# linuxstb/dabtools

Hardware: AMD Instinct MI355X
Metric: ETI frames/s (24 ms each), Mode-I batch, synthetic IQ resident in HBM (higher is better)
Workload: dtype f64 sync / f32 OFDM / u16 ACS / u8 ETI

## Files before the change

### dabtools_amd/csrc/fft64.hpp

```cpp
#pragma once

#include <hip/hip_runtime.h>

namespace dabhip {
namespace {

constexpr int kFft64Threads = 512;

__device__ __forceinline__ unsigned brev(unsigned x, int bits) { return __brev(x) >> (32 - bits); }

__device__ __forceinline__ int lds_at(int i) { return i ^ ((i >> 3) & 7) ^ ((i >> 6) & 7); }

template <class V>
struct ScalarOf;
template <>
struct ScalarOf<double2> { using type = double; };
template <>
struct ScalarOf<float2> { using type = float; };

template <int LOGN, int L, class V>
__device__ __forceinline__ void dif_levels(V* buf, int nbatch, int s, typename ScalarOf<V>::type sign, const V* tw2048)
{
  using R = typename ScalarOf<V>::type;
  constexpr int N = 1 << LOGN, RADIX = 1 << L;
  const int ms = N >> s;
  const int q = ms >> L;
  constexpr int per_batch = N >> L;
  for (int idx = threadIdx.x; idx < nbatch * per_batch; idx += kFft64Threads) {
    const int batch = idx / per_batch, w = idx % per_batch;
    const int blk = w / q, k = w % q;
    const int e0 = batch * N + blk * ms + k;
    V r[RADIX];
#pragma unroll
    for (int j = 0; j < RADIX; ++j) r[j] = buf[lds_at(e0 + j * q)];
#pragma unroll
    for (int l = 0; l < L; ++l) {
      const int span = RADIX >> (l + 1);
      const int half = ms >> (l + 1);
      const int twstep = 1024 / half;
#pragma unroll
      for (int j = 0; j < RADIX; ++j) {
        if (j & span) continue;
        const int pos = k + (j & (span - 1)) * q;
        const V A = r[j], B = r[j + span];
        V tw = tw2048[lds_at(pos * twstep)];
        tw.y *= sign;
        const R dr = A.x - B.x, di = A.y - B.y;
        r[j].x = A.x + B.x;
        r[j].y = A.y + B.y;
        r[j + span].x = dr * tw.x - di * tw.y;
        r[j + span].y = dr * tw.y + di * tw.x;
      }
    }
#pragma unroll
    for (int j = 0; j < RADIX; ++j) buf[lds_at(e0 + j * q)] = r[j];
  }
  __syncthreads();
}

template <int LOGN, int... Ls, class V>
__device__ __forceinline__ void dft_dif(V* buf, int nbatch, typename ScalarOf<V>::type sign, const V* tw2048)
{
  int s = 0;
  ((dif_levels<LOGN, Ls>(buf, nbatch, s, sign, tw2048), s += Ls), ...);
}

}
}
```

### dabtools_amd/csrc/k_sync.hip

```cpp
#include <hip/hip_runtime.h>

#include <algorithm>
#include <cstdlib>
#include <type_traits>

#include "dab_tables.hpp"
#include "device_types.hpp"
#include "fft64.hpp"
#include "fifo_view.hpp"
#include "kernels.hpp"

namespace dabhip {
namespace {

constexpr int kThreads = kFft64Threads;

#ifndef DABHIP_SYNC_TIMES
#define DABHIP_SYNC_TIMES 0
#endif
#ifndef DABHIP_K1_TAIL
#define DABHIP_K1_TAIL 1
#endif
#if DABHIP_SYNC_TIMES
__device__ unsigned long long g_sync_times[96 * 16];
__device__ volatile int g_sync_call;
#define SYNC_STAMP(i) do { if (blockIdx.x == 0 && threadIdx.x == 0 && g_sync_call < 96) g_sync_times[g_sync_call * 16 + (i)] = wall_clock64(); } while (0)
#else
#define SYNC_STAMP(i) do {} while (0)
#endif

__device__ __forceinline__ int view_byte(const uint8_t* stream, const FrameView& v, int p) { return frame_byte(stream, v, p); }
__device__ __forceinline__ double2 view_sample(const uint8_t* stream, const FrameView& v, int p, int nco_hz)
{
  const unsigned w = frame_u16(stream, v, p);
  const double2 x = make_double2(static_cast<int8_t>(static_cast<uint8_t>((w & 0xff) - 127)), static_cast<int8_t>(static_cast<uint8_t>((w >> 8) - 127)));
  if (nco_hz == 0) return x;
  double sn, cs;
  sincospi(-2.0 * nco_hz * (p >> 1) / 2048000.0, &sn, &cs);
  return make_double2(x.x * cs - x.y * sn, x.x * sn + x.y * cs);
}
__device__ __forceinline__ int rail(int byte) { return static_cast<int>(static_cast<int8_t>(static_cast<uint8_t>(byte - 127))); }

__device__ __forceinline__ const uint8_t* contiguous_window(const uint8_t* stream, const FrameView& v, int p0, int p1)
{
  return (v.seg_src[0] >= 0 && p1 <= v.seg_end[0]) ? stream + v.seg_src[0] + p0 : nullptr;
}
__device__ __forceinline__ double2 sample_of(unsigned w)
{
  return make_double2(static_cast<int8_t>(static_cast<uint8_t>((w & 0xff) - 127)), static_cast<int8_t>(static_cast<uint8_t>((w >> 8) - 127)));
}
template <int kCount>
struct Prefetched {
  bool ok;
  unsigned w[kCount / kThreads];
};
template <int kCount>
__device__ __forceinline__ Prefetched<kCount> prefetch_samples(const uint8_t* stream, const FrameView& view, int p0, int nco)
{
  Prefetched<kCount> pf;
  const uint8_t* win = nco == 0 ? contiguous_window(stream, view, p0, p0 + 2 * kCount) : nullptr;
  pf.ok = win != nullptr;
  if (pf.ok) {
    const uint16_t* src = reinterpret_cast<const uint16_t*>(win);
#pragma unroll
    for (int i = 0; i < kCount / kThreads; ++i) pf.w[i] = src[threadIdx.x + i * kThreads];
  }
  return pf;
}
template <int kCount>
__device__ __forceinline__ void load_samples(const uint8_t* stream, const FrameView& view, int p0, int nco, double2* dst)
{
  const int tid = threadIdx.x;
  const uint8_t* win = nco == 0 ? contiguous_window(stream, view, p0, p0 + 2 * kCount) : nullptr;
  if (win) {
    const uint16_t* src = reinterpret_cast<const uint16_t*>(win);
    unsigned w[kCount / kThreads];
#pragma unroll
    for (int i = 0; i < kCount / kThreads; ++i) w[i] = src[tid + i * kThreads];
#pragma unroll
    for (int i = 0; i < kCount / kThreads; ++i) dst[lds_at(tid + i * kThreads)] = sample_of(w[i]);
  } else {
    for (int n = tid; n < kCount; n += kThreads) dst[lds_at(n)] = view_sample(stream, view, p0 + 2 * n, nco);
  }
}

constexpr int kWaves = kThreads / 64;
struct Red {
  float fv[kWaves];
  int iv[kWaves];
  double dv[kWaves];
};

template <int kCtrl, int kRowMask>
__device__ __forceinline__ int dpp_from(int own)
{
  return __builtin_amdgcn_update_dpp(own, own, kCtrl, kRowMask, 0xf, false);
}
template <typename F>
__device__ __forceinline__ void wave_reduce_steps(F&& step)
{
  step(std::integral_constant<int, 0xB1>{}, std::integral_constant<int, 0xf>{});
  step(std::integral_constant<int, 0x4E>{}, std::integral_constant<int, 0xf>{});
  step(std::integral_constant<int, 0x141>{}, std::integral_constant<int, 0xf>{});
  step(std::integral_constant<int, 0x140>{}, std::integral_constant<int, 0xf>{});
  step(std::integral_constant<int, 0x142>{}, std::integral_constant<int, 0xa>{});
  step(std::integral_constant<int, 0x143>{}, std::integral_constant<int, 0xc>{});
}

__device__ void block_argmax(Red& r, float v, int idx, float* out_v, int* out_i)
{
  wave_reduce_steps([&](auto ctrl, auto mask) {
    const float ov = __builtin_bit_cast(float, dpp_from<decltype(ctrl)::value, decltype(mask)::value>(__builtin_bit_cast(int, v)));
    const int oi = dpp_from<decltype(ctrl)::value, decltype(mask)::value>(idx);
    if (ov > v || (ov == v && oi < idx)) { v = ov; idx = oi; }
  });
  if ((threadIdx.x & 63) == 63) { r.fv[threadIdx.x >> 6] = v; r.iv[threadIdx.x >> 6] = idx; }
  __syncthreads();
  float bv = r.fv[0];
  int bi = r.iv[0];
#pragma unroll
  for (int w = 1; w < kWaves; ++w) {
    const float ov = r.fv[w];
    const int oi = r.iv[w];
    if (ov > bv || (ov == bv && oi < bi)) { bv = ov; bi = oi; }
  }
  *out_v = bv;
  *out_i = bi;
  __syncthreads();
}

__device__ int block_sum_int(Red& r, int v)
{
  wave_reduce_steps([&](auto ctrl, auto mask) {
    v += __builtin_amdgcn_update_dpp(0, v, decltype(ctrl)::value, decltype(mask)::value, 0xf, false);
  });
  if ((threadIdx.x & 63) == 63) r.iv[threadIdx.x >> 6] = v;
  __syncthreads();
  int out = 0;
#pragma unroll
  for (int w = 0; w < kWaves; ++w) out += r.iv[w];
  __syncthreads();
  return out;
}

__device__ double block_sum_double(Red& r, double v)
{
  wave_reduce_steps([&](auto ctrl, auto mask) {
    const long long bits = __builtin_bit_cast(long long, v);
    const int lo = __builtin_amdgcn_update_dpp(0, static_cast<int>(bits), decltype(ctrl)::value, decltype(mask)::value, 0xf, false);
    const int hi = __builtin_amdgcn_update_dpp(0, static_cast<int>(bits >> 32), decltype(ctrl)::value, decltype(mask)::value, 0xf, false);
    v += __builtin_bit_cast(double, (static_cast<long long>(hi) << 32) | static_cast<unsigned>(lo));
  });
  if ((threadIdx.x & 63) == 63) r.dv[threadIdx.x >> 6] = v;
  __syncthreads();
  double out = 0;
#pragma unroll
  for (int w = 0; w < kWaves; ++w) out += r.dv[w];
  __syncthreads();
  return out;
}

__device__ __forceinline__ double2 mul_conj_prs(double2 x, int q)
{
  switch (q & 3) {
    case 0: return x;
    case 1: return make_double2(x.y, -x.x);
    case 2: return make_double2(-x.x, -x.y);
    default: return make_double2(-x.y, x.x);
  }
}

struct Shared {
  StreamState st;
  Red red;
  int status, do_sync, fifo_count, fresh;
  int coarse_fs;
  double fine_fs;
  int2 ahead;
};

constexpr int kBatchPoints = 29 * 128 - 2048;
constexpr int kSpecBins = 128 + 28;


__device__ __forceinline__ int null_symbol_energy_part(const uint8_t* stream, const FrameView& view)
{
  const int tid = threadIdx.x;
  int e = 0;
  if (const uint8_t* win = contiguous_window(stream, view, 0, 20 * 266)) {
    if (tid < 266) e = abs(rail(win[20 * tid]));
  } else {
    for (int n = tid; n < 266; n += kThreads) e += abs(rail(view_byte(stream, view, 20 * n)));
  }
  return e;
}
__device__ int coarse_time_search(const uint8_t* stream, const FrameView& view, Red& red, uint8_t* env)
{
  const int tid = threadIdx.x;
  constexpr int kEnv = (kTfSamples - kNullSamples) / 10 + 266;
  constexpr int kWin = (kTfSamples - kNullSamples) / 10;
  for (int n = tid; n < kEnv; n += kThreads) env[n] = static_cast<uint8_t>(abs(rail(view_byte(stream, view, 20 * n))));
  __syncthreads();
  const int per = (kWin + kThreads - 1) / kThreads;
  const int m0 = tid * per, m1 = min(m0 + per, kWin);
  float best = 9999999.0f;
  int bestm = 0x7fffffff;
  if (m0 < m1) {
    int s = 0;
    for (int q = 0; q < 266; ++q) s += env[m0 + q];
    for (int m = m0; m < m1; ++m) {
      if (static_cast<float>(s) < best) { best = static_cast<float>(s); bestm = m; }
      s += env[m + 266] - env[m];
    }
  }
  float bv;
  int bi;
  block_argmax(red, -best, bestm, &bv, &bi);
  const int coarse = (-bv < 9999999.0f) ? bi * 20 : 0;
  __syncthreads();
  return coarse;
}

struct FineTimeTables {
  int q[3];
  double2 w1[3], w2[3];
};
__device__ __forceinline__ FineTimeTables fine_time_tables(const double2* __restrict__ tw1536, const uint8_t* __restrict__ prs_q)
{
  static_assert(kCarriers == 3 * kThreads, "three carriers per thread");
  FineTimeTables t;
#pragma unroll
  for (int j = 0; j < 3; ++j) {
    const int i = threadIdx.x + j * kThreads;
    t.q[j] = prs_q[i];
    t.w1[j] = tw1536[i];
    t.w2[j] = tw1536[(2 * i) % 1536];
  }
  return t;
}

__device__ int fine_time_sync(const uint8_t* stream, const FrameView& view, int nco, double2* A, double2* Bf, const double2* tw,
                              const FineTimeTables& tab, Red& red, const Prefetched<2048>& pf)
{
  const int tid = threadIdx.x;
  if (pf.ok) {
#pragma unroll
    for (int i = 0; i < 2048 / kThreads; ++i) A[lds_at(tid + i * kThreads)] = sample_of(pf.w[i]);
  } else {
    load_samples<2048>(stream, view, 2 * (kNullSamples + kCpSamples), nco, A);
  }
  __syncthreads();
  SYNC_STAMP(3);
  dft_dif<11, 3, 3, 3, 2>(A, 1, -1.0, tw);
  SYNC_STAMP(4);
#pragma unroll
  for (int j = 0; j < 3; ++j) {
    const int i = tid + j * kThreads;
    const int bin = i < 768 ? i + 1280 : i - 765;
    const double2 c = mul_conj_prs(A[lds_at(brev(bin, 11))], tab.q[j]);
    Bf[lds_at((i % 3) * 512 + i / 3)] = c;
  }
  __syncthreads();
  SYNC_STAMP(5);
  dft_dif<9, 3, 3, 3>(Bf, 3, +1.0, tw);
  SYNC_STAMP(6);
  float fv = -99999.0f;
  int fi = 0x7fffffff;
#pragma unroll
  for (int j = 0; j < 3; ++j) {
    const int kk = tid + j * kThreads;
    const int r = brev(kk & 511, 9);
    const double2 f0 = Bf[lds_at(r)], f1 = Bf[lds_at(512 + r)], f2 = Bf[lds_at(1024 + r)];
    const double2 w1 = tab.w1[j], w2 = tab.w2[j];
    const double xr = f0.x + (f1.x * w1.x - f1.y * w1.y) + (f2.x * w2.x - f2.y * w2.y);
    const double xi = f0.y + (f1.x * w1.y + f1.y * w1.x) + (f2.x * w2.y + f2.y * w2.x);
    const float mag = static_cast<float>(sqrt(xr * xr + xi * xi));
    if (mag > fv) { fv = mag; fi = kk; }
  }
  float gv;
  int gi;
  SYNC_STAMP(7);
  block_argmax(red, fv, fi, &gv, &gi);
  SYNC_STAMP(8);
  return gi < 768 ? gi * 2 + 16 : (gi - 1536) * 2;
}

__device__ int coarse_freq_sync(const uint8_t* stream, const FrameView& view, int nco, int fine, double2* A, double2* spec, const double2* tw,
                                const uint8_t* __restrict__ prs_q, Red& red)
{
  const int tid = threadIdx.x;
  load_samples<2048>(stream, view, 2 * (kNullSamples + kCpSamples + 1 + fine), nco, A);
  __syncthreads();
  dft_dif<11, 3, 3, 3, 2>(A, 1, -1.0, tw);
  for (int j = tid; j < kSpecBins; j += kThreads) spec[j] = A[lds_at(brev((256 + j + 1024) & 2047, 11))];
  __syncthreads();
  double2* W = A;
  for (int idx = tid; idx < 29 * 128; idx += kThreads) {
    const int o = idx / 128, s = idx % 128;
    W[lds_at(idx)] = mul_conj_prs(spec[o + s], prs_q[14 + s]);
  }
  __syncthreads();
  dft_dif<7, 3, 2, 2>(W, 29, +1.0, tw);
  float cv = -99999.0f;
  int ci = 0x7fffffff;
  for (int idx = tid; idx < 29 * 128; idx += kThreads) {
    const double2 x = W[lds_at(idx)];
    const float mag = static_cast<float>(sqrt(x.x * x.x + x.y * x.y));
    if (mag > cv) { cv = mag; ci = idx / 128; }
  }
  float hv;
  int hi;
  block_argmax(red, cv, ci, &hv, &hi);
  return hi - 14;
}

constexpr int kVerifyAgain = 0x7fff0000;
__device__ __forceinline__ float2 mul_conj_prs32(float2 x, int q)
{
  switch (q & 3) {
    case 0: return x;
    case 1: return make_float2(x.y, -x.x);
    case 2: return make_float2(-x.x, -x.y);
    default: return make_float2(-x.y, x.x);
  }
}
__device__ int coarse_freq_sync32(const uint8_t* stream, const FrameView& view, int fine, float2* A, float2* spec, const float2* tw,
                                  const uint8_t* __restrict__ prs_q, Red& red, bool* clear)
{
  const int tid = threadIdx.x;
  {
    const int p0 = 2 * (kNullSamples + kCpSamples + 1 + fine);
    if (const uint8_t* win = contiguous_window(stream, view, p0, p0 + 2 * 2048)) {
      const uint16_t* src = reinterpret_cast<const uint16_t*>(win);
      unsigned w[2048 / kThreads];
#pragma unroll
// ... 42 lines not shown
  float ov = 0.0f;
#pragma unroll
  for (int k = 0; k < kPer; ++k)
    if ((tid + k * kThreads) / 128 != hi) ov = fmaxf(ov, mags[k]);
  float rv;
  int ri;
  block_argmax(red, ov, tid, &rv, &ri);
  *clear = hv > 0.0f && (hv - rv) > 0.01f * hv;
  return hi - 14;
}

__device__ double fine_freq_corr(const uint8_t* stream, const FrameView& view, int nco, Red& red)
{
  double acc = 0;
  const uint8_t* win = nco == 0 ? contiguous_window(stream, view, 2 * kNullSamples, 2 * (kNullSamples + 2048 + kCpSamples)) : nullptr;
  for (int n = threadIdx.x; n < kCpSamples; n += kThreads) {
    const int pl = 2 * (kNullSamples + 2048 + n), pr = 2 * (kNullSamples + n);
    double2 l, r;
    if (win) {
      const uint16_t* src = reinterpret_cast<const uint16_t*>(win);
      l = sample_of(src[2048 + n]);
      r = sample_of(src[n]);
    } else {
      l = view_sample(stream, view, pl, nco);
      r = view_sample(stream, view, pr, nco);
    }
    const double lr = l.x, li = l.y, rr = r.x, ri = r.y;
    acc += atan2(-lr * ri + li * rr, lr * rr + li * ri);
  }
  acc = block_sum_double(red, acc);
  return acc / 504 / (2 * M_PI) * 1000;
}

struct SyncLds {
  double2* A;
  double2* Bf;
  double2* tw;
  double2* spec;
  Shared* sh;
};
__device__ __forceinline__ SyncLds sync_lds(unsigned char* smem, const double2* __restrict__ tw2048, bool fill = true)
{
  SyncLds l;
  l.A = reinterpret_cast<double2*>(smem);
  l.Bf = l.A + 2048;
  l.tw = l.Bf + kBatchPoints;
  l.spec = l.tw + 1024;
  l.sh = reinterpret_cast<Shared*>(l.spec + kSpecBins);
  if (fill)
    for (int i = threadIdx.x; i < 1024; i += kThreads) l.tw[lds_at(i)] = tw2048[i];
  return l;
}

__device__ __forceinline__ void fifo_call_wave(Shared& sh, int chunk, const uint8_t* tail_slot)
{
  const int lane = threadIdx.x;
  StreamState& st = sh.st;
  const int64_t fed = st.fed + chunk;
  int64_t consumed = st.consumed, count = fed - consumed;
  int status = 0, do_sync = 0, fresh = 0;
  int startup = st.startup_delay;
  if (count >= 3 * kTfSamples) {
    const int shift = st.coarse_timeshift + st.fine_timeshift;
    const int64_t consumed0 = consumed;
    int len, skipped = 0;
    if (shift > 0) {
      consumed += shift;
      count -= shift;
      len = count < kTfBytes ? static_cast<int>(count) : kTfBytes;
      skipped = shift;
    } else {
      len = kTfBytes + shift;
    }
    const bool extra = skipped > len;
    const int n0 = extra ? 2 : 1, covered = extra ? skipped : len;
    const int old_n = st.view.nseg;
    const int old_end = lane < kMaxSeg ? st.view.seg_end[lane] : 0;
    const int prev_end = lane > 0 && lane < kMaxSeg ? st.view.seg_end[lane - 1] : 0;
    const int64_t old_src = lane < kMaxSeg ? st.view.seg_src[lane] : -1;
    const bool keep = lane < old_n && lane < kMaxSeg && old_end > covered && covered < kTailStart && prev_end < kTailStart;
    fresh = n0;
    const unsigned long long mask = __ballot(keep);
    const int pos = n0 + __popcll(mask & ((1ull << lane) - 1ull));
    const int total = n0 + __popcll(mask);
    const int n = total < kMaxSeg ? total : kMaxSeg;
    if (keep && pos < kMaxSeg) { st.view.seg_end[pos] = old_end; st.view.seg_src[pos] = old_src; }
    if (lane >= n && lane < kMaxSeg) { st.view.seg_end[lane] = kTfBytes; st.view.seg_src[lane] = -1; }
    if (lane == 0) {
      st.view.seg_end[0] = len;
      st.view.seg_src[0] = consumed;
      if (extra) { st.view.seg_end[1] = skipped; st.view.seg_src[1] = consumed0; }
      st.view.nseg = n;
      st.view.tail = tail_slot;
      if (total > kMaxSeg) st.overflow = 1;
    }
    consumed += len;
    count -= len;
    status = 1;
    if (startup <= 0) ++startup;
    else do_sync = 1;
  }
  if (lane == 0) {
    st.fed = fed;
    st.consumed = consumed;
    st.startup_delay = startup;
    sh.status = status;
    sh.do_sync = do_sync;
    sh.fifo_count = static_cast<int>(count);
    sh.fresh = fresh;
    sh.coarse_fs = 0;
  }
}

struct CallEnv {
  const uint8_t* stream;
  int b, max_calls, kdesc0, afc;
  CallDesc* descs;
  int2* info;
  SyncTails tails;
  SyncLds lds;
  const uint8_t* prs_q;
  bool ahead;
  const int2* ahead_table;
  const int64_t* ahead_src0;
  int* ahead_hits;
  int ahead_nspec, ahead_nhyp;
  int kahead0;
};
struct TailUpdate {
  unsigned lo = 0, hi = 0;
  bool take_lo = false, take_hi = false;
};
constexpr int kTailWords = kTailBytes / 4;
__device__ __forceinline__ TailUpdate tail_load(const uint8_t* stream, const Shared& sh, bool frame_read)
{
  TailUpdate u;
  const int tid = threadIdx.x;
  if (frame_read && tid < kTailWords) {
    const int64_t s0 = read_source(sh.st.view, sh.fresh, kTailStart + 4 * tid), s1 = read_source(sh.st.view, sh.fresh, kTailStart + 4 * tid + 2);
    u.take_lo = s0 >= 0;
    u.take_hi = s1 >= 0;
    if (u.take_lo) u.lo = *reinterpret_cast<const uint16_t*>(stream + s0);
    if (u.take_hi) u.hi = *reinterpret_cast<const uint16_t*>(stream + s1);
  }
  return u;
}
__device__ __forceinline__ void tail_commit(const TailUpdate& u, bool frame_read, uint32_t& tail_word, uint8_t* tail_slot)
{
  const int tid = threadIdx.x;
  if (frame_read && tid < kTailWords) {
    if (u.take_lo) tail_word = (tail_word & 0xffff0000u) | u.lo;
    if (u.take_hi) tail_word = (tail_word & 0x0000ffffu) | (u.hi << 16);
    if (tail_slot) reinterpret_cast<uint32_t*>(tail_slot)[tid] = tail_word;
  }
}

constexpr int kAheadWindowEnd = 2 * (kNullSamples + kCpSamples) + 2 * 2048;
struct AheadRow {
  int64_t src0 = -1;
  int2 entry = make_int2(-1, 0);
};
__device__ __forceinline__ AheadRow ahead_fetch(const int2* __restrict__ table, const int64_t* __restrict__ src0, int nspec, int nhyp, int b, int j)
{
  AheadRow r;
  if (j >= 0 && j < nspec) {
    const size_t slot = static_cast<size_t>(b) * nspec + j;
    r.src0 = src0[slot];
    if (static_cast<int>(threadIdx.x) < nhyp) r.entry = table[slot * nhyp + threadIdx.x];
  }
  return r;
}
__device__ __forceinline__ int2 ahead_lookup(int nhyp, const AheadRow& row, const FrameView& view)
{
  const int2 miss = make_int2(-1, 0);
  const int64_t src = view.seg_src[0];
  if (row.src0 < 0 || src < 0 || view.seg_end[0] < kAheadWindowEnd) return miss;
  const int64_t d = src - row.src0;
  const int half = nhyp / 2;
  if ((d & 1) != 0 || d < -2 * half || d > 2 * half) return miss;
  const int h = static_cast<int>(d / 2) + half;
  return make_int2(__shfl(row.entry.x, h), __shfl(row.entry.y, h));
}
struct TailPending {
  TailUpdate upd;
  uint8_t* slot = nullptr;
  bool valid = false;
};
template <bool kChainOnly>
__device__ __forceinline__ void sync_call(const CallEnv& env, Shared& sh, int k, const FineTimeTables& fine_tab, uint32_t& tail_word, AheadRow& row, TailPending& pend)
{
  const int tid = threadIdx.x;
  if (pend.valid) {
    tail_commit(pend.upd, true, tail_word, pend.slot);
    pend.valid = false;
  }
  const uint8_t* const stream = env.stream;
  double2* const A = env.lds.A;
  double2* const Bf = env.lds.Bf;
  double2* const tw = env.lds.tw;
  uint8_t* const env_bytes = reinterpret_cast<uint8_t*>(Bf);
  SYNC_STAMP(0);
  uint8_t* const tail_slot = env.tails.images ? env.tails.images + (static_cast<size_t>(env.b) * env.max_calls + (k - env.kdesc0)) * kTailBytes : nullptr;
  if (tid < 64) {
    fifo_call_wave(sh, env.tails.chunk, tail_slot);
    if (env.ahead) {
      const int2 found = sh.do_sync ? ahead_lookup(env.ahead_nhyp, row, sh.st.view) : make_int2(-1, 0);
      if (tid == 0) sh.ahead = found;
      row = ahead_fetch(env.ahead_table, env.ahead_src0, env.ahead_nspec, env.ahead_nhyp, env.b, k + 1 - env.kahead0);
    }
  }
  __syncthreads();

  const bool frame_read = DABHIP_K1_TAIL && sh.status != 0;
  TailUpdate tail_upd;

  const int nco = env.afc ? sh.st.tuner_hz : 0;
  if (sh.do_sync) {
    const FrameView& view = sh.st.view;
    const int2 ahead = env.ahead ? sh.ahead : make_int2(-1, 0);
    const bool hit = ahead.x >= 0;
    if (hit && tid == 0) atomicAdd(env.ahead_hits, 1);
    Prefetched<2048> pf;
    pf.ok = false;
    if (!hit) pf = prefetch_samples<2048>(stream, view, 2 * (kNullSamples + kCpSamples), nco);
    SYNC_STAMP(1);
    const int force = sh.st.force_timesync;
    const int energy_part = hit ? 0 : null_symbol_energy_part(stream, view);
    tail_upd = tail_load(stream, sh, frame_read);
    int energy = ahead.x;
    if (hit) __syncthreads();
    else energy = block_sum_int(sh.red, energy_part);
    if (hit && frame_read && energy < 5000 && force == 0) {
      pend.upd = tail_upd;
      pend.slot = tail_slot;
      pend.valid = true;
    } else {
      tail_commit(tail_upd, frame_read, tail_word, tail_slot);
    }
    int coarse = 0;
    if (energy >= 5000 || force != 0) {
      __syncthreads();
      coarse = coarse_time_search(stream, view, sh.red, env_bytes);
    }
    if (tid == 0) { sh.st.coarse_timeshift = coarse; sh.st.force_timesync = 0; }
    __syncthreads();
    SYNC_STAMP(2);
    if (coarse == 0) {
      const int fine = hit ? ahead.y : fine_time_sync(stream, view, nco, A, Bf, tw, fine_tab, sh.red, pf);
      if (tid == 0) sh.st.fine_timeshift = fine;
      if (kChainOnly) {
        if (tid == 0) sh.status = 2;
      } else {
        const int cfs = coarse_freq_sync(stream, view, nco, fine, A, env.lds.spec, tw, env.prs_q, sh.red);
        if (tid == 0) sh.coarse_fs = cfs;
        if (abs(cfs) > 1) {
          if (tid == 0) sh.st.force_timesync = 1;
        } else {
          const double ffs = fine_freq_corr(stream, view, nco, sh.red);
          if (tid == 0) {
            sh.fine_fs = ffs;
            sh.status = 2;
          }
        }
      }
    }
  } else {
    tail_upd = tail_load(stream, sh, frame_read);
    tail_commit(tail_upd, frame_read, tail_word, tail_slot);
  }
  __syncthreads();
  if (tid >= 64 && tid < 64 + static_cast<int>(sizeof(FrameView) / 4)) {
    CallDesc& d = env.descs[static_cast<size_t>(env.b) * env.max_calls + (k - env.kdesc0)];
    reinterpret_cast<uint32_t*>(&d.view)[tid - 64] = reinterpret_cast<const uint32_t*>(&sh.st.view)[tid - 64];
  }
  if (tid == 0) {
    CallDesc& d = env.descs[static_cast<size_t>(env.b) * env.max_calls + (k - env.kdesc0)];
    d.status = sh.status;
    d.ordinal = sh.status == 2 ? sh.st.next_ordinal++ : -1;
    if (env.info) env.info[static_cast<size_t>(env.b) * env.max_calls + (k - env.kdesc0)] = make_int2(d.status, d.ordinal);
    d.coarse_timeshift = sh.st.coarse_timeshift;
    d.fine_timeshift = sh.st.fine_timeshift;
    d.coarse_freq_shift = sh.coarse_fs;
    d.fifo_count = sh.fifo_count;
    d.fine_freq_shift = sh.fine_fs;
    d.nco_hz = nco;
    if (env.afc) {
      StreamState& st = sh.st;
      const int c = sh.coarse_fs;
      if (abs(c) > 1) st.tuner_hz += c < 0 ? -1000 : 1000;
      if (abs(c) == 1) {
        st.rng = st.rng * 1103515245u + 12345u;
        const int step = static_cast<int>((st.rng >> 16) % 1000u);
        st.tuner_hz += c < 0 ? -step : step;
      }
      if (c == 0 && abs(static_cast<int>(sh.fine_fs)) > 50) st.tuner_hz += static_cast<int>(floor(sh.fine_fs / 3));
    }
  }
  __syncthreads();
  SYNC_STAMP(9);
}

template <bool kChainOnly>
__global__ __launch_bounds__(kThreads) void sync_scan_kernel(const uint8_t* const* __restrict__ iq,
                                                             const int64_t* __restrict__ nbytes,
                                                             const StreamState* __restrict__ states_in, StreamState* __restrict__ states,
                                                             const int* __restrict__ stream_list,
                                                             CallDesc* __restrict__ descs, int2* __restrict__ info, int max_calls, int call_begin,
                                                             int call_end, const double2* __restrict__ tw2048,
                                                             const double2* __restrict__ tw1536,
                                                             const uint8_t* __restrict__ prs_q, int afc, SyncTails tails, SpecArgs spec)
{
  extern __shared__ __attribute__((aligned(16))) unsigned char smem[];
  const int b = stream_list ? stream_list[blockIdx.x] : blockIdx.x, tid = threadIdx.x;
  const int64_t total_calls = nbytes[b] / kChunkBytes;
  int kend = call_end < 0 ? static_cast<int>(total_calls) : min(call_end, static_cast<int>(total_calls));
  const int kfirst = call_begin >= 0 ? call_begin : static_cast<int>(states_in[b].fed / kChunkBytes);
  int kdesc0 = call_begin >= 0 ? 0 : kfirst;
  if (spec.ctl) {
    if (spec.record_base) { if (tid == 0) { spec.ctl[b] = kdesc0; if (blockIdx.x == 0) spec.ctl[gridDim.x] = 0; } }
    else kdesc0 = spec.ctl[b];
  }
  if (spec.call_limit >= 0) kend = min(kend, kfirst + spec.call_limit);
  if (spec.call_limit >= 0 && kfirst >= kend) return;
  const SyncLds lds = sync_lds(smem, tw2048);
  Shared& sh = *lds.sh;
  const CallEnv env{iq[b], b, max_calls, kdesc0, afc, descs, info, tails, lds, prs_q, spec.lookup != 0, spec.table, spec.src0, spec.ctl + spec.nstreams, spec.nspec, spec.nhyp, kfirst};
  if (tid == 0) { sh.st = states_in[b]; sh.fine_fs = sh.st.fine_freq_shift; }
  const FineTimeTables fine_tab = fine_time_tables(tw1536, prs_q);
  uint32_t tail_word = 0;
  if (tails.state_in && tid < kTailWords) tail_word = reinterpret_cast<const uint32_t*>(tails.state_in + static_cast<size_t>(b) * kTailBytes)[tid];
  __syncthreads();

  AheadRow row;
  TailPending pend;
  if (env.ahead && tid < 64) row = ahead_fetch(env.ahead_table, env.ahead_src0, env.ahead_nspec, env.ahead_nhyp, b, 0);
  for (int k = kfirst; k < kend; ++k) {
#if DABHIP_SYNC_TIMES
    if (blockIdx.x == 0 && tid == 0) g_sync_call = k - kfirst;
#endif
    sync_call<kChainOnly>(env, sh, k, fine_tab, tail_word, row, pend);
  }
  if (pend.valid) tail_commit(pend.upd, true, tail_word, pend.slot);
  if (tid == 0) { sh.st.fine_freq_shift = sh.fine_fs; states[b] = sh.st; }
  if (tails.state_out && tid < kTailWords) reinterpret_cast<uint32_t*>(tails.state_out + static_cast<size_t>(b) * kTailBytes)[tid] = tail_word;
}

__global__ __launch_bounds__(kThreads) void sync_ahead_kernel(const uint8_t* const* __restrict__ iq, const int64_t* __restrict__ nbytes,
                                                              const StreamState* __restrict__ states, const double2* __restrict__ tw2048,
                                                              const double2* __restrict__ tw1536, const uint8_t* __restrict__ prs_q, int chunk, SpecArgs spec)
{
  extern __shared__ __attribute__((aligned(16))) unsigned char smem[];
  const int b = blockIdx.z, j = blockIdx.y, h = blockIdx.x, tid = threadIdx.x;
  const int total_calls = static_cast<int>(nbytes[b] / kChunkBytes);
  const int kcur = static_cast<int>(states[b].fed / kChunkBytes);
  if (j >= min(spec.nspec, total_calls - kcur)) return;
  const SyncLds lds = sync_lds(smem, tw2048, false);
  Shared& sh = *lds.sh;
  static_assert(sizeof(StreamState) % 4 == 0 && sizeof(StreamState) / 4 <= kThreads, "copied word by word");
  if (tid < static_cast<int>(sizeof(StreamState) / 4)) reinterpret_cast<uint32_t*>(&sh.st)[tid] = reinterpret_cast<const uint32_t*>(states + b)[tid];
  __syncthreads();

  int i = 0;
  while (i < j) {
    const bool lean = sh.st.coarse_timeshift + sh.st.fine_timeshift == 0 && sh.st.startup_delay > 0 && chunk == kChunkBytes;
    __syncthreads();
    if (!lean) {
      if (tid < 64) fifo_call_wave(sh, chunk, nullptr);
      __syncthreads();
      if (tid == 0 && sh.do_sync) {
        sh.st.coarse_timeshift = sh.st.fine_timeshift = sh.st.force_timesync = 0;
        ++sh.st.next_ordinal;
      }
      __syncthreads();
      ++i;
      continue;
    }
    int64_t fed = sh.st.fed, consumed = sh.st.consumed;
    fifo_skip_unshifted(fed, consumed, j - i);
    i = j;
    if (tid == 0) { sh.st.fed = fed; sh.st.consumed = consumed; }
    __syncthreads();
  }

  if (tid < 64) fifo_call_wave(sh, chunk, nullptr);
  __syncthreads();
  const bool expected = sh.do_sync && sh.st.view.seg_src[0] >= 0 && sh.st.view.seg_end[0] >= kAheadWindowEnd;
  const int64_t src0 = expected ? sh.st.view.seg_src[0] : -1;
  const size_t slot = static_cast<size_t>(b) * spec.nspec + j;
  if (h == 0 && tid == 0) spec.src0[slot] = src0;
  if (!expected) return;
  const int64_t src = src0 + 2 * (h - spec.nhyp / 2);
  int2 out = make_int2(-1, 0);
  if (src >= 0 && src + kAheadWindowEnd <= nbytes[b]) {
    const FineTimeTables fine_tab = fine_time_tables(tw1536, prs_q);
    for (int n = tid; n < 1024; n += kThreads) lds.tw[lds_at(n)] = tw2048[n];
// ... 76 lines not shown
  bool clear;
  const int cfs = coarse_freq_sync32(stream, sh.st.view, fine, A, spec, tw, prs_q, sh.red, &clear);
  if (!clear || distrust) {
    if (threadIdx.x == 0) { d.coarse_freq_shift = kVerifyAgain; atomicAdd(violation + nstreams, 1); }
    return;
  }
  if (abs(cfs) > 1) {
    if (threadIdx.x == 0) { d.coarse_freq_shift = cfs; atomicMin(violation + b, w % max_calls); }
    return;
  }
  const double ffs = fine_freq_corr(stream, sh.st.view, 0, sh.red);
  if (threadIdx.x == 0) { d.coarse_freq_shift = cfs; d.fine_freq_shift = ffs; }
}

__global__ __launch_bounds__(256) void sync_carry_kernel(CallDesc* __restrict__ descs, int max_calls, const int64_t* __restrict__ nbytes, const int* __restrict__ calls_before,
                                                         StreamState* __restrict__ states, const int* __restrict__ violation, int nstreams)
{
  const int b = blockIdx.x * 4 + (threadIdx.x >> 6), lane = threadIdx.x & 63;
  if (b >= nstreams || violation[b] != 0x7f7f7f7f) return;
  const int ncalls = static_cast<int>(nbytes[b] / kChunkBytes) - calls_before[b];
  double carried = states[b].fine_freq_shift;
  for (int k0 = 0; k0 < ncalls; k0 += 64) {
    const int k = k0 + lane;
    CallDesc* d = descs + static_cast<size_t>(b) * max_calls + k;
    const bool valid = k < ncalls, demod = valid && d->status == 2;
    const double own = demod ? d->fine_freq_shift : 0.0;
    const unsigned long long mask = __ballot(demod);
    const unsigned long long earlier = mask & ((lane == 63) ? ~0ull : ((2ull << lane) - 1ull));
    const int src = earlier ? 63 - __clzll(earlier) : -1;
    const long long bits = __builtin_bit_cast(long long, own);
    const int lo = __shfl(static_cast<int>(bits), src < 0 ? 0 : src), hi = __shfl(static_cast<int>(bits >> 32), src < 0 ? 0 : src);
    const double v = src < 0 ? carried : __builtin_bit_cast(double, (static_cast<long long>(hi) << 32) | static_cast<unsigned>(lo));
    if (valid && !demod) d->fine_freq_shift = v;
    if (mask) {
      const int last = 63 - __clzll(mask);
      const int l2 = __shfl(static_cast<int>(bits), last), h2 = __shfl(static_cast<int>(bits >> 32), last);
      carried = __builtin_bit_cast(double, (static_cast<long long>(h2) << 32) | static_cast<unsigned>(l2));
    }
  }
  if (lane == 0) states[b].fine_freq_shift = carried;
}

}

size_t sync_scan_lds_bytes() { return sizeof(double2) * (2048 + kBatchPoints + 1024 + kSpecBins) + sizeof(Shared); }
static size_t sync_verify32_lds_bytes() { return sizeof(float2) * (kVerify32Points + 1024 + kSpecBins + (kSpecBins & 1)) + sizeof(Shared); }

static hipError_t sync_attr()
{
  static std::once_flag once[64];
  static hipError_t result[64];
  return once_per_device(once, result, []() {
    const int lds = static_cast<int>(sync_scan_lds_bytes());
    hipError_t e = hipFuncSetAttribute(reinterpret_cast<const void*>(sync_scan_kernel<false>), hipFuncAttributeMaxDynamicSharedMemorySize, lds);
    if (e == hipSuccess) e = hipFuncSetAttribute(reinterpret_cast<const void*>(sync_scan_kernel<true>), hipFuncAttributeMaxDynamicSharedMemorySize, lds);
    if (e == hipSuccess) e = hipFuncSetAttribute(reinterpret_cast<const void*>(sync_ahead_kernel), hipFuncAttributeMaxDynamicSharedMemorySize, lds);
    if (e == hipSuccess) e = hipFuncSetAttribute(reinterpret_cast<const void*>(sync_verify_kernel), hipFuncAttributeMaxDynamicSharedMemorySize, lds);
    if (e == hipSuccess) e = hipFuncSetAttribute(reinterpret_cast<const void*>(sync_verify32_kernel), hipFuncAttributeMaxDynamicSharedMemorySize, static_cast<int>(sync_verify32_lds_bytes()));
    return e;
  });
}

namespace {
__global__ __launch_bounds__(256) void scan_setup_kernel(ScanSetupArgs a)
{
  const size_t tid = static_cast<size_t>(blockIdx.x) * blockDim.x + threadIdx.x, step = static_cast<size_t>(gridDim.x) * blockDim.x;
  const uint4 zero = make_uint4(0, 0, 0, 0);
  for (size_t i = tid; i < a.desc_vec; i += step) a.descs[i] = zero;
  for (size_t i = tid; i < a.info_vec; i += step) a.info[i] = zero;
  constexpr size_t kStateWords = sizeof(StreamState) / 4;
  const size_t nstate_words = static_cast<size_t>(a.nstreams) * kStateWords;
  const uint32_t* src = reinterpret_cast<const uint32_t*>(a.h_states ? a.h_states : a.states);
  for (size_t i = tid; i < nstate_words; i += step) {
    const uint32_t w = src[i];
    if (a.h_states) reinterpret_cast<uint32_t*>(a.states)[i] = w;
    if (a.states_prev) reinterpret_cast<uint32_t*>(a.states_prev)[i] = w;
  }
  if (a.tail_state) {
    const size_t ntail_words = static_cast<size_t>(a.nstreams) * (kTailBytes / 4);
    for (size_t i = tid; i < ntail_words; i += step) {
      const uint32_t w = a.h_states ? 0u : reinterpret_cast<const uint32_t*>(a.tail_state)[i];
      if (a.h_states) reinterpret_cast<uint32_t*>(a.tail_state)[i] = 0u;
      if (a.tail_state_prev) reinterpret_cast<uint32_t*>(a.tail_state_prev)[i] = w;
    }
  }
  for (size_t b = tid; b < static_cast<size_t>(a.nstreams); b += step) {
    a.iq_ptrs[b] = a.h_ptrs[b];
    a.nbytes[b] = a.h_nbytes[b];
    if (a.calls_before) a.calls_before[b] = a.h_calls_before[b];
    if (a.viol) a.viol[b] = 0x7f7f7f7f;
  }
  if (tid == 0 && a.viol) a.viol[a.nstreams] = 0;
}
}
namespace {
__global__ __launch_bounds__(256) void host_words_kernel(HostWordsArgs a)
{
  const uint32_t tid = blockIdx.x * blockDim.x + threadIdx.x, step = gridDim.x * blockDim.x;
#pragma unroll
  for (int k = 0; k < 4; ++k)
    for (uint32_t i = tid; i < a.nwords[k]; i += step) a.dst[k][i] = a.src[k][i];
  for (uint32_t i = tid; i < a.nzero; i += step) a.zero[i] = 0;
}
}
hipError_t launch_host_words(const HostWordsArgs& a, hipStream_t stream)
{
  uint32_t most = a.nzero;
  for (int k = 0; k < 4; ++k) most = most > a.nwords[k] ? most : a.nwords[k];
  if (most == 0) return hipSuccess;
  const int blocks = static_cast<int>(most / 256 + 1 > 256 ? 256 : most / 256 + 1);
  hipLaunchKernelGGL(host_words_kernel, dim3(blocks), dim3(256), 0, stream, a);
  return hipGetLastError();
}

hipError_t launch_scan_setup(const ScanSetupArgs& a, hipStream_t stream)
{
  static_assert(sizeof(StreamState) % 4 == 0, "copied word by word");
  const size_t most = a.desc_vec > a.info_vec ? a.desc_vec : a.info_vec;
  const int blocks = static_cast<int>(most / 256 / 4 < 64 ? 64 : (most / 256 / 4 > 2048 ? 2048 : most / 256 / 4));
  hipLaunchKernelGGL(scan_setup_kernel, dim3(blocks), dim3(256), 0, stream, a);
  return hipGetLastError();
}

hipError_t launch_sync_scan(const uint8_t* const* iq, const int64_t* nbytes, StreamState* states, CallDesc* descs, int2* info,
                            int nstreams, int max_calls, int call_begin, int call_end, const double2* tw2048,
                            const double2* tw1536, const uint8_t* prs_q, int afc, hipStream_t stream, bool chain_only,
                            const StreamState* states_in, const int* stream_list, SyncTails tails, SpecArgs spec)
{
  if (tails.chunk < 0) tails.chunk = kChunkBytes;
  if (nstreams <= 0) return hipSuccess;
  hipError_t e = sync_attr();
  if (e != hipSuccess) return e;
  const size_t lds = sync_scan_lds_bytes();
  if (!states_in) states_in = states;
  if (chain_only)
    hipLaunchKernelGGL(sync_scan_kernel<true>, dim3(nstreams), dim3(kThreads), lds, stream, iq, nbytes, states_in, states, stream_list, descs, info,
                       max_calls, call_begin, call_end, tw2048, tw1536, prs_q, afc, tails, spec);
  else
    hipLaunchKernelGGL(sync_scan_kernel<false>, dim3(nstreams), dim3(kThreads), lds, stream, iq, nbytes, states_in, states, stream_list, descs, info,
                       max_calls, call_begin, call_end, tw2048, tw1536, prs_q, afc, tails, spec);
  return hipGetLastError();
}

hipError_t launch_sync_ahead(const uint8_t* const* iq, const int64_t* nbytes, const StreamState* states, int nstreams, const double2* tw2048, const double2* tw1536,
                             const uint8_t* prs_q, hipStream_t stream, const SpecArgs& spec)
{
  if (nstreams <= 0 || spec.nspec <= 0 || spec.nhyp <= 0) return hipSuccess;
  hipError_t e = sync_attr();
  if (e != hipSuccess) return e;
  hipLaunchKernelGGL(sync_ahead_kernel, dim3(spec.nhyp, spec.nspec, nstreams), dim3(kThreads), sync_scan_lds_bytes(), stream, iq, nbytes, states, tw2048, tw1536, prs_q,
                     kChunkBytes, spec);
  return hipGetLastError();
}

hipError_t launch_sync_verify(const uint8_t* const* iq, const int64_t* nbytes, const int* calls_before, StreamState* states, CallDesc* descs,
                              int nstreams, int max_calls, const double2* tw2048, const uint8_t* prs_q, int* violation, bool carry_only, hipStream_t stream)
{
  if (nstreams <= 0 || max_calls <= 0) return hipSuccess;
  hipError_t e = sync_attr();
  if (e != hipSuccess) return e;
  if (!carry_only) {
    const int blocks = max_calls * nstreams;
    static const int mode = std::getenv("DABHIP_VERIFY_FP32") ? std::atoi(std::getenv("DABHIP_VERIFY_FP32")) : 1;
    const bool fp32_first = mode != 0;
    if (fp32_first)
      hipLaunchKernelGGL(sync_verify32_kernel, dim3(blocks), dim3(kThreads), sync_verify32_lds_bytes(), stream, iq, descs, max_calls, nstreams, tw2048, prs_q, violation,
                         mode == 2 ? 1 : 0);
    hipLaunchKernelGGL(sync_verify_kernel, dim3(fp32_first ? std::min(blocks, 1024) : blocks), dim3(kThreads), sync_scan_lds_bytes(), stream, iq, descs, max_calls,
                       nstreams, tw2048, prs_q, violation, fp32_first ? 1 : 0);
  } else {
    hipLaunchKernelGGL(sync_carry_kernel, dim3((nstreams + 3) / 4), dim3(256), 0, stream, descs, max_calls, nbytes, calls_before, states, violation, nstreams);
  }
  return hipGetLastError();
}


#if DABHIP_SYNC_TIMES
}
extern "C" int dabhip_debug_sync_times(unsigned long long* out)
{
  return hipMemcpyFromSymbol(out, HIP_SYMBOL(dabhip::g_sync_times), sizeof(unsigned long long) * 96 * 16) == hipSuccess ? 0 : -1;
}
namespace dabhip {
#endif
}
```

Baseline: 4.768 million.

## Overlap next-call FIFO bookkeeping with sync tail and drop redundant barriers

Moves the per-call FIFO and ahead-table bookkeeping from the start of each sync call to the end of the previous one, so it shares that call's final barrier instead of needing its own. Removes the trailing barriers in the argmax and sum reductions where the caller already synchronises. Adds a specialised chain-only variant with no ahead lookup and a higher occupancy launch bound. Passes the thread id explicitly so the compiler can assume its range. This reduces barrier count and register pressure in the serial sync scan. It risks LDS reuse races from the removed barriers, and chain-only calls with AFC enabled now return an error.

Measured after the change: 4.736 million, median of 2. Within noise of the previous version (-0.7%).

```diff
diff --git a/dabtools_amd/csrc/fft64.hpp b/dabtools_amd/csrc/fft64.hpp
--- a/dabtools_amd/csrc/fft64.hpp
+++ b/dabtools_amd/csrc/fft64.hpp
@@ -19,14 +19,14 @@
 struct ScalarOf<float2> { using type = float; };
 
 template <int LOGN, int L, class V>
-__device__ __forceinline__ void dif_levels(V* buf, int nbatch, int s, typename ScalarOf<V>::type sign, const V* tw2048)
+__device__ __forceinline__ void dif_levels(V* buf, int nbatch, int s, typename ScalarOf<V>::type sign, const V* tw2048, int tid)
 {
   using R = typename ScalarOf<V>::type;
   constexpr int N = 1 << LOGN, RADIX = 1 << L;
   const int ms = N >> s;
   const int q = ms >> L;
   constexpr int per_batch = N >> L;
-  for (int idx = threadIdx.x; idx < nbatch * per_batch; idx += kFft64Threads) {
+  for (int idx = tid; idx < nbatch * per_batch; idx += kFft64Threads) {
     const int batch = idx / per_batch, w = idx % per_batch;
     const int blk = w / q, k = w % q;
     const int e0 = batch * N + blk * ms + k;
@@ -59,10 +59,10 @@
 }
 
 template <int LOGN, int... Ls, class V>
-__device__ __forceinline__ void dft_dif(V* buf, int nbatch, typename ScalarOf<V>::type sign, const V* tw2048)
+__device__ __forceinline__ void dft_dif(V* buf, int nbatch, typename ScalarOf<V>::type sign, const V* tw2048, int tid = threadIdx.x)
 {
   int s = 0;
-  ((dif_levels<LOGN, Ls>(buf, nbatch, s, sign, tw2048), s += Ls), ...);
+  ((dif_levels<LOGN, Ls>(buf, nbatch, s, sign, tw2048, tid), s += Ls), ...);
 }
 
 }
diff --git a/dabtools_amd/csrc/k_sync.hip b/dabtools_amd/csrc/k_sync.hip
--- a/dabtools_amd/csrc/k_sync.hip
+++ b/dabtools_amd/csrc/k_sync.hip
@@ -55,7 +55,7 @@
   unsigned w[kCount / kThreads];
 };
 template <int kCount>
-__device__ __forceinline__ Prefetched<kCount> prefetch_samples(const uint8_t* stream, const FrameView& view, int p0, int nco)
+__device__ __forceinline__ Prefetched<kCount> prefetch_samples(const uint8_t* stream, const FrameView& view, int p0, int nco, int tid = threadIdx.x)
 {
   Prefetched<kCount> pf;
   const uint8_t* win = nco == 0 ? contiguous_window(stream, view, p0, p0 + 2 * kCount) : nullptr;
@@ -63,14 +63,13 @@
   if (pf.ok) {
     const uint16_t* src = reinterpret_cast<const uint16_t*>(win);
 #pragma unroll
-    for (int i = 0; i < kCount / kThreads; ++i) pf.w[i] = src[threadIdx.x + i * kThreads];
+    for (int i = 0; i < kCount / kThreads; ++i) pf.w[i] = src[tid + i * kThreads];
   }
   return pf;
 }
 template <int kCount>
-__device__ __forceinline__ void load_samples(const uint8_t* stream, const FrameView& view, int p0, int nco, double2* dst)
-{
-  const int tid = threadIdx.x;
+__device__ __forceinline__ void load_samples(const uint8_t* stream, const FrameView& view, int p0, int nco, double2* dst, int tid = threadIdx.x)
+{
   const uint8_t* win = nco == 0 ? contiguous_window(stream, view, p0, p0 + 2 * kCount) : nullptr;
   if (win) {
     const uint16_t* src = reinterpret_cast<const uint16_t*>(win);
@@ -107,14 +106,15 @@
   step(std::integral_constant<int, 0x143>{}, std::integral_constant<int, 0xc>{});
 }
 
-__device__ void block_argmax(Red& r, float v, int idx, float* out_v, int* out_i)
+template <bool kRelease = true>
+__device__ void block_argmax(Red& r, float v, int idx, float* out_v, int* out_i, int tid = threadIdx.x)
 {
   wave_reduce_steps([&](auto ctrl, auto mask) {
     const float ov = __builtin_bit_cast(float, dpp_from<decltype(ctrl)::value, decltype(mask)::value>(__builtin_bit_cast(int, v)));
     const int oi = dpp_from<decltype(ctrl)::value, decltype(mask)::value>(idx);
     if (ov > v || (ov == v && oi < idx)) { v = ov; idx = oi; }
   });
-  if ((threadIdx.x & 63) == 63) { r.fv[threadIdx.x >> 6] = v; r.iv[threadIdx.x >> 6] = idx; }
+  if ((tid & 63) == 63) { r.fv[tid >> 6] = v; r.iv[tid >> 6] = idx; }
   __syncthreads();
   float bv = r.fv[0];
   int bi = r.iv[0];
@@ -126,20 +126,21 @@
   }
   *out_v = bv;
   *out_i = bi;
-  __syncthreads();
-}
-
-__device__ int block_sum_int(Red& r, int v)
+  if (kRelease) __syncthreads();
+}
+
+template <bool kRelease = true>
+__device__ int block_sum_int(Red& r, int v, int tid = threadIdx.x)
 {
   wave_reduce_steps([&](auto ctrl, auto mask) {
     v += __builtin_amdgcn_update_dpp(0, v, decltype(ctrl)::value, decltype(mask)::value, 0xf, false);
   });
-  if ((threadIdx.x & 63) == 63) r.iv[threadIdx.x >> 6] = v;
+  if ((tid & 63) == 63) r.iv[tid >> 6] = v;
   __syncthreads();
   int out = 0;
 #pragma unroll
   for (int w = 0; w < kWaves; ++w) out += r.iv[w];
-  __syncthreads();
+  if (kRelease) __syncthreads();
   return out;
 }
 
@@ -183,9 +184,8 @@
 constexpr int kSpecBins = 128 + 28;
 
 
-__device__ __forceinline__ int null_symbol_energy_part(const uint8_t* stream, const FrameView& view)
-{
-  const int tid = threadIdx.x;
+__device__ __forceinline__ int null_symbol_energy_part(const uint8_t* stream, const FrameView& view, int tid = threadIdx.x)
+{
   int e = 0;
   if (const uint8_t* win = contiguous_window(stream, view, 0, 20 * 266)) {
     if (tid < 266) e = abs(rail(win[20 * tid]));
@@ -194,9 +194,8 @@
   }
   return e;
 }
-__device__ int coarse_time_search(const uint8_t* stream, const FrameView& view, Red& red, uint8_t* env)
-{
-  const int tid = threadIdx.x;
+__device__ int coarse_time_search(const uint8_t* stream, const FrameView& view, Red& red, uint8_t* env, int tid = threadIdx.x)
+{
   constexpr int kEnv = (kTfSamples - kNullSamples) / 10 + 266;
   constexpr int kWin = (kTfSamples - kNullSamples) / 10;
   for (int n = tid; n < kEnv; n += kThreads) env[n] = static_cast<uint8_t>(abs(rail(view_byte(stream, view, 20 * n))));
@@ -215,7 +214,7 @@
   }
   float bv;
   int bi;
-  block_argmax(red, -best, bestm, &bv, &bi);
+  block_argmax(red, -best, bestm, &bv, &bi, tid);
   const int coarse = (-bv < 9999999.0f) ? bi * 20 : 0;
   __syncthreads();
   return coarse;
@@ -240,18 +239,17 @@
 }
 
 __device__ int fine_time_sync(const uint8_t* stream, const FrameView& view, int nco, double2* A, double2* Bf, const double2* tw,
-                              const FineTimeTables& tab, Red& red, const Prefetched<2048>& pf)
-{
-  const int tid = threadIdx.x;
+                              const FineTimeTables& tab, Red& red, const Prefetched<2048>& pf, int tid = threadIdx.x)
+{
   if (pf.ok) {
 #pragma unroll
     for (int i = 0; i < 2048 / kThreads; ++i) A[lds_at(tid + i * kThreads)] = sample_of(pf.w[i]);
   } else {
-    load_samples<2048>(stream, view, 2 * (kNullSamples + kCpSamples), nco, A);
+    load_samples<2048>(stream, view, 2 * (kNullSamples + kCpSamples), nco, A, tid);
   }
   __syncthreads();
   SYNC_STAMP(3);
-  dft_dif<11, 3, 3, 3, 2>(A, 1, -1.0, tw);
+  dft_dif<11, 3, 3, 3, 2>(A, 1, -1.0, tw, tid);
   SYNC_STAMP(4);
 #pragma unroll
   for (int j = 0; j < 3; ++j) {
@@ -262,7 +260,7 @@
   }
   __syncthreads();
   SYNC_STAMP(5);
-  dft_dif<9, 3, 3, 3>(Bf, 3, +1.0, tw);
+  dft_dif<9, 3, 3, 3>(Bf, 3, +1.0, tw, tid);
   SYNC_STAMP(6);
   float fv = -99999.0f;
   int fi = 0x7fffffff;
@@ -280,7 +278,7 @@
   float gv;
   int gi;
   SYNC_STAMP(7);
-  block_argmax(red, fv, fi, &gv, &gi);
+  block_argmax<false>(red, fv, fi, &gv, &gi, tid);
   SYNC_STAMP(8);
   return gi < 768 ? gi * 2 + 16 : (gi - 1536) * 2;
 }
@@ -429,9 +427,8 @@
   return l;
 }
 
-__device__ __forceinline__ void fifo_call_wave(Shared& sh, int chunk, const uint8_t* tail_slot)
-{
-  const int lane = threadIdx.x;
+__device__ __forceinline__ void fifo_call_wave(Shared& sh, int chunk, const uint8_t* tail_slot, int lane = threadIdx.x)
+{
   StreamState& st = sh.st;
   const int64_t fed = st.fed + chunk;
   int64_t consumed = st.consumed, count = fed - consumed;
@@ -509,10 +506,9 @@
   bool take_lo = false, take_hi = false;
 };
 constexpr int kTailWords = kTailBytes / 4;
-__device__ __forceinline__ TailUpdate tail_load(const uint8_t* stream, const Shared& sh, bool frame_read)
+__device__ __forceinline__ TailUpdate tail_load(const uint8_t* stream, const Shared& sh, bool frame_read, int tid = threadIdx.x)
 {
   TailUpdate u;
-  const int tid = threadIdx.x;
   if (frame_read && tid < kTailWords) {
     const int64_t s0 = read_source(sh.st.view, sh.fresh, kTailStart + 4 * tid), s1 = read_source(sh.st.view, sh.fresh, kTailStart + 4 * tid + 2);
     u.take_lo = s0 >= 0;
@@ -522,9 +518,8 @@
   }
   return u;
 }
-__device__ __forceinline__ void tail_commit(const TailUpdate& u, bool frame_read, uint32_t& tail_word, uint8_t* tail_slot)
-{
-  const int tid = threadIdx.x;
+__device__ __forceinline__ void tail_commit(const TailUpdate& u, bool frame_read, uint32_t& tail_word, uint8_t* tail_slot, int tid = threadIdx.x)
+{
   if (frame_read && tid < kTailWords) {
     if (u.take_lo) tail_word = (tail_word & 0xffff0000u) | u.lo;
     if (u.take_hi) tail_word = (tail_word & 0x0000ffffu) | (u.hi << 16);
@@ -563,12 +558,28 @@
   uint8_t* slot = nullptr;
   bool valid = false;
 };
-template <bool kChainOnly>
-__device__ __forceinline__ void sync_call(const CallEnv& env, Shared& sh, int k, const FineTimeTables& fine_tab, uint32_t& tail_word, AheadRow& row, TailPending& pend)
-{
-  const int tid = threadIdx.x;
-  if (pend.valid) {
-    tail_commit(pend.upd, true, tail_word, pend.slot);
+__device__ __forceinline__ uint8_t* call_tail_slot(const CallEnv& env, int k)
+{
+  return env.tails.images ? env.tails.images + (static_cast<size_t>(env.b) * env.max_calls + (k - env.kdesc0)) * kTailBytes : nullptr;
+}
+template <bool kAhead>
+__device__ __forceinline__ void call_bookkeeping(const CallEnv& env, Shared& sh, int k, AheadRow& row, int tid)
+{
+  fifo_call_wave(sh, env.tails.chunk, call_tail_slot(env, k), tid);
+  if (kAhead && env.ahead) {
+    const int2 found = sh.do_sync ? ahead_lookup(env.ahead_nhyp, row, sh.st.view) : make_int2(-1, 0);
+    if (tid == 0) sh.ahead = found;
+    row = ahead_fetch(env.ahead_table, env.ahead_src0, env.ahead_nspec, env.ahead_nhyp, env.b, k + 1 - env.kahead0);
+  }
+}
+template <bool kChainOnly, bool kAhead>
+__device__ __forceinline__ void sync_call(const CallEnv& env, Shared& sh, int k, int kend, const FineTimeTables& fine_tab, uint32_t& tail_word, AheadRow& row, TailPending& pend)
+{
+  int tid = threadIdx.x;
+  if (kChainOnly) asm volatile("" : "+v"(tid));
+  __builtin_assume(tid >= 0 && tid < kThreads);
+  if (kAhead && pend.valid) {
+    tail_commit(pend.upd, true, tail_word, pend.slot, tid);
     pend.valid = false;
   }
   const uint8_t* const stream = env.stream;
@@ -577,53 +588,44 @@
   double2* const tw = env.lds.tw;
   uint8_t* const env_bytes = reinterpret_cast<uint8_t*>(Bf);
   SYNC_STAMP(0);
-  uint8_t* const tail_slot = env.tails.images ? env.tails.images + (static_cast<size_t>(env.b) * env.max_calls + (k - env.kdesc0)) * kTailBytes : nullptr;
-  if (tid < 64) {
-    fifo_call_wave(sh, env.tails.chunk, tail_slot);
-    if (env.ahead) {
-      const int2 found = sh.do_sync ? ahead_lookup(env.ahead_nhyp, row, sh.st.view) : make_int2(-1, 0);
-      if (tid == 0) sh.ahead = found;
-      row = ahead_fetch(env.ahead_table, env.ahead_src0, env.ahead_nspec, env.ahead_nhyp, env.b, k + 1 - env.kahead0);
-    }
-  }
-  __syncthreads();
+  uint8_t* const tail_slot = call_tail_slot(env, k);
 
   const bool frame_read = DABHIP_K1_TAIL && sh.status != 0;
   TailUpdate tail_upd;
 
-  const int nco = env.afc ? sh.st.tuner_hz : 0;
+  const int nco = !kChainOnly && env.afc ? sh.st.tuner_hz : 0;
   if (sh.do_sync) {
     const FrameView& view = sh.st.view;
-    const int2 ahead = env.ahead ? sh.ahead : make_int2(-1, 0);
+    const int2 ahead = kAhead && env.ahead ? sh.ahead : make_int2(-1, 0);
     const bool hit = ahead.x >= 0;
     if (hit && tid == 0) atomicAdd(env.ahead_hits, 1);
     Prefetched<2048> pf;
     pf.ok = false;
-    if (!hit) pf = prefetch_samples<2048>(stream, view, 2 * (kNullSamples + kCpSamples), nco);
+    if (!hit) pf = prefetch_samples<2048>(stream, view, 2 * (kNullSamples + kCpSamples), nco, tid);
     SYNC_STAMP(1);
     const int force = sh.st.force_timesync;
-    const int energy_part = hit ? 0 : null_symbol_energy_part(stream, view);
-    tail_upd = tail_load(stream, sh, frame_read);
+    const int energy_part = hit ? 0 : null_symbol_energy_part(stream, view, tid);
+    tail_upd = tail_load(stream, sh, frame_read, tid);
     int energy = ahead.x;
     if (hit) __syncthreads();
-    else energy = block_sum_int(sh.red, energy_part);
+    else energy = block_sum_int<false>(sh.red, energy_part, tid);
     if (hit && frame_read && energy < 5000 && force == 0) {
       pend.upd = tail_upd;
       pend.slot = tail_slot;
       pend.valid = true;
     } else {
-      tail_commit(tail_upd, frame_read, tail_word, tail_slot);
+      tail_commit(tail_upd, frame_read, tail_word, tail_slot, tid);
     }
     int coarse = 0;
     if (energy >= 5000 || force != 0) {
       __syncthreads();
-      coarse = coarse_time_search(stream, view, sh.red, env_bytes);
+      coarse = coarse_time_search(stream, view, sh.red, env_bytes, tid);
     }
     if (tid == 0) { sh.st.coarse_timeshift = coarse; sh.st.force_timesync = 0; }
     __syncthreads();
     SYNC_STAMP(2);
     if (coarse == 0) {
-      const int fine = hit ? ahead.y : fine_time_sync(stream, view, nco, A, Bf, tw, fine_tab, sh.red, pf);
+      const int fine = hit ? ahead.y : fine_time_sync(stream, view, nco, A, Bf, tw, fine_tab, sh.red, pf, tid);
       if (tid == 0) sh.st.fine_timeshift = fine;
       if (kChainOnly) {
         if (tid == 0) sh.status = 2;
@@ -642,13 +644,14 @@
       }
     }
   } else {
-    tail_upd = tail_load(stream, sh, frame_read);
-    tail_commit(tail_upd, frame_read, tail_word, tail_slot);
-  }
-  __syncthreads();
-  if (tid >= 64 && tid < 64 + static_cast<int>(sizeof(FrameView) / 4)) {
+    tail_upd = tail_load(stream, sh, frame_read, tid);
+    tail_commit(tail_upd, frame_read, tail_word, tail_slot, tid);
+  }
+  __syncthreads();
+  static_assert(sizeof(FrameView) / 4 <= 64, "the view, word by word, by one wave");
+  if (tid < static_cast<int>(sizeof(FrameView) / 4)) {
     CallDesc& d = env.descs[static_cast<size_t>(env.b) * env.max_calls + (k - env.kdesc0)];
-    reinterpret_cast<uint32_t*>(&d.view)[tid - 64] = reinterpret_cast<const uint32_t*>(&sh.st.view)[tid - 64];
+    reinterpret_cast<uint32_t*>(&d.view)[tid] = reinterpret_cast<const uint32_t*>(&sh.st.view)[tid];
   }
   if (tid == 0) {
     CallDesc& d = env.descs[static_cast<size_t>(env.b) * env.max_calls + (k - env.kdesc0)];
@@ -661,7 +664,7 @@
     d.fifo_count = sh.fifo_count;
     d.fine_freq_shift = sh.fine_fs;
     d.nco_hz = nco;
-    if (env.afc) {
+    if (!kChainOnly && env.afc) {
       StreamState& st = sh.st;
       const int c = sh.coarse_fs;
       if (abs(c) > 1) st.tuner_hz += c < 0 ? -1000 : 1000;
@@ -673,12 +676,13 @@
       if (c == 0 && abs(static_cast<int>(sh.fine_fs)) > 50) st.tuner_hz += static_cast<int>(floor(sh.fine_fs / 3));
     }
   }
+  if (tid < 64 && k + 1 < kend) call_bookkeeping<kAhead>(env, sh, k + 1, row, tid);
   __syncthreads();
   SYNC_STAMP(9);
 }
 
-template <bool kChainOnly>
-__global__ __launch_bounds__(kThreads) void sync_scan_kernel(const uint8_t* const* __restrict__ iq,
+template <bool kChainOnly, bool kAhead>
+__global__ __launch_bounds__(kThreads, (kChainOnly && !kAhead) ? 4 : 2) void sync_scan_kernel(const uint8_t* const* __restrict__ iq,
                                                              const int64_t* __restrict__ nbytes,
                                                              const StreamState* __restrict__ states_in, StreamState* __restrict__ states,
                                                              const int* __restrict__ stream_list,
@@ -710,14 +714,18 @@
 
   AheadRow row;
   TailPending pend;
-  if (env.ahead && tid < 64) row = ahead_fetch(env.ahead_table, env.ahead_src0, env.ahead_nspec, env.ahead_nhyp, b, 0);
+  if (kAhead && env.ahead && tid < 64) row = ahead_fetch(env.ahead_table, env.ahead_src0, env.ahead_nspec, env.ahead_nhyp, b, 0);
+  if (kfirst < kend) {
+    if (tid < 64) call_bookkeeping<kAhead>(env, sh, kfirst, row, tid);
+    __syncthreads();
+  }
   for (int k = kfirst; k < kend; ++k) {
 #if DABHIP_SYNC_TIMES
     if (blockIdx.x == 0 && tid == 0) g_sync_call = k - kfirst;
 #endif
-    sync_call<kChainOnly>(env, sh, k, fine_tab, tail_word, row, pend);
-  }
-  if (pend.valid) tail_commit(pend.upd, true, tail_word, pend.slot);
+    sync_call<kChainOnly, kAhead>(env, sh, k, kend, fine_tab, tail_word, row, pend);
+  }
+  if (kAhead && pend.valid) tail_commit(pend.upd, true, tail_word, pend.slot);
   if (tid == 0) { sh.st.fine_freq_shift = sh.fine_fs; states[b] = sh.st; }
   if (tails.state_out && tid < kTailWords) reinterpret_cast<uint32_t*>(tails.state_out + static_cast<size_t>(b) * kTailBytes)[tid] = tail_word;
 }
@@ -900,8 +908,9 @@
   static hipError_t result[64];
   return once_per_device(once, result, []() {
     const int lds = static_cast<int>(sync_scan_lds_bytes());
-    hipError_t e = hipFuncSetAttribute(reinterpret_cast<const void*>(sync_scan_kernel<false>), hipFuncAttributeMaxDynamicSharedMemorySize, lds);
-    if (e == hipSuccess) e = hipFuncSetAttribute(reinterpret_cast<const void*>(sync_scan_kernel<true>), hipFuncAttributeMaxDynamicSharedMemorySize, lds);
+    hipError_t e = hipFuncSetAttribute(reinterpret_cast<const void*>(sync_scan_kernel<false, true>), hipFuncAttributeMaxDynamicSharedMemorySize, lds);
+    if (e == hipSuccess) e = hipFuncSetAttribute(reinterpret_cast<const void*>(sync_scan_kernel<true, true>), hipFuncAttributeMaxDynamicSharedMemorySize, lds);
+    if (e == hipSuccess) e = hipFuncSetAttribute(reinterpret_cast<const void*>(sync_scan_kernel<true, false>), hipFuncAttributeMaxDynamicSharedMemorySize, lds);
     if (e == hipSuccess) e = hipFuncSetAttribute(reinterpret_cast<const void*>(sync_ahead_kernel), hipFuncAttributeMaxDynamicSharedMemorySize, lds);
     if (e == hipSuccess) e = hipFuncSetAttribute(reinterpret_cast<const void*>(sync_verify_kernel), hipFuncAttributeMaxDynamicSharedMemorySize, lds);
     if (e == hipSuccess) e = hipFuncSetAttribute(reinterpret_cast<const void*>(sync_verify32_kernel), hipFuncAttributeMaxDynamicSharedMemorySize, static_cast<int>(sync_verify32_lds_bytes()));
@@ -981,11 +990,15 @@
   if (e != hipSuccess) return e;
   const size_t lds = sync_scan_lds_bytes();
   if (!states_in) states_in = states;
-  if (chain_only)
-    hipLaunchKernelGGL(sync_scan_kernel<true>, dim3(nstreams), dim3(kThreads), lds, stream, iq, nbytes, states_in, states, stream_list, descs, info,
+  if (chain_only && afc) return hipErrorInvalidValue;
+  if (chain_only && spec.lookup != 0)
+    hipLaunchKernelGGL((sync_scan_kernel<true, true>), dim3(nstreams), dim3(kThreads), lds, stream, iq, nbytes, states_in, states, stream_list, descs, info,
+                       max_calls, call_begin, call_end, tw2048, tw1536, prs_q, afc, tails, spec);
+  else if (chain_only)
+    hipLaunchKernelGGL((sync_scan_kernel<true, false>), dim3(nstreams), dim3(kThreads), lds, stream, iq, nbytes, states_in, states, stream_list, descs, info,
                        max_calls, call_begin, call_end, tw2048, tw1536, prs_q, afc, tails, spec);
   else
-    hipLaunchKernelGGL(sync_scan_kernel<false>, dim3(nstreams), dim3(kThreads), lds, stream, iq, nbytes, states_in, states, stream_list, descs, info,
+    hipLaunchKernelGGL((sync_scan_kernel<false, true>), dim3(nstreams), dim3(kThreads), lds, stream, iq, nbytes, states_in, states, stream_list, descs, info,
                        max_calls, call_begin, call_end, tw2048, tw1536, prs_q, afc, tails, spec);
   return hipGetLastError();
 }
```
